# megapose6d/megapose6d

Measured on NVIDIA H100. Metric: pose hypotheses/sec through render+coarse+5x refine, higher is better.
Workload: dtype f16

## Files before the change

### include/mpx.h

```cpp
#ifndef MPX_H_
#define MPX_H_

#include <stddef.h>
#include <stdint.h>

#ifdef __cplusplus
extern "C" {
#endif

#define MPX_ABI_VERSION 5

int mpx_abi_version(void);
int mpx_act_dtype(void);
const char* mpx_last_error(void);
long long mpx_launch_count(void);
int mpx_set_sm_limit(int n_sms);
int mpx_sm_count(void);
int mpx_profile_enable(int on);
int mpx_profile_summary(double* conv_ms, double* conv_flops, long long* conv_launches);

typedef struct mpx_meshdb mpx_meshdb;
int mpx_meshdb_create(int n_meshes, const float* h_verts, const float* h_normals,
                      const float* h_colors, const int64_t* h_vert_offsets, const int32_t* h_faces,
                      const int64_t* h_face_offsets, mpx_meshdb** out);
// ... 37 lines not shown
                          int c_in, void* d_x, int c_pad, int ch_per_view, const float* d_depth_norm_z,
                          void* d_workspace, size_t workspace_bytes, void* stream);

int mpx_pose_init_autodepth(const float* d_points, int n_pts, const int32_t* d_label_idx,
                            const float* d_bboxes, const float* d_K, const float* d_R, int n,
                            float* d_TCO, void* stream);

int mpx_normalize_T(const float* d_T_in, int n, float* d_T_out, void* stream);

int mpx_crop_geometry(const float* d_points, int n_pts, const int32_t* d_label_idx,
                      const float* d_TCO, const float* d_K, const float* d_tCR, int n, float lamb,
                      int im_h, int im_w, int out_h, int out_w, float* d_boxes_rend,
                      float* d_boxes_crop, float* d_K_crop, void* stream);

int mpx_multiview_cameras(const float* d_TCO, const float* d_tCR, int n, const float* h_offsets,
                          int n_extra, float* d_TCV_O, void* stream);

int mpx_pose_update(const float* d_TCO, const float* d_K_crop, const float* d_pose9,
                    const float* d_tCR, int n, float* d_TCO_out, void* stream);

int mpx_topk_per_group(const float* d_logits, int n_groups, int m, int k, int32_t* d_idx,
                       void* stream);

int mpx_image_to_nhwc4(const float* d_images_nchw, int b, int c, int h, int w, float* d_out_nhwc4,
                       void* stream);
int mpx_roi_align(const float* d_img_nhwc4, int b, int h, int w, const int32_t* d_im_idx,
                  const float* d_boxes, int n, int c, int out_h, int out_w, float* d_out,
                  void* stream);
int mpx_roi_align_fused(const float* d_img_nhwc4, int b, int h, int w, const int32_t* d_im_idx,
                        const float* d_boxes, int n, int c, int out_h, int out_w, void* d_x,
                        int c_pad, const float* d_depth_norm_z, int depth_norm_kind, void* stream);

size_t mpx_net_input_bytes(int n, int h, int w, int c_pad);

int mpx_conv2d(const void* d_x, int n, int h, int w, int c_in, const void* d_w,
                    const float* d_bias, int c_out, int r, int s, int stride, int pad_lo_h,
                    int pad_lo_w, int pad_hi_h, int pad_hi_w, int relu, const void* d_residual,
                    void* d_out, int block_n, int max_ctas, void* stream);

int mpx_conv2d_splitk(const void* d_x, int n, int h, int w, int c_in, const void* d_w,
                           const float* d_bias, int c_out, int r, int s, int stride, int pad_lo_h,
                           int pad_lo_w, int pad_hi_h, int pad_hi_w, int relu, const void* d_residual,
                           void* d_out, int block_n, int splits, void* stream);

#define MPX_CONV_NET_SPLITK 8
#define MPX_CONV_NO_PDL 512
#define MPX_CONV_SPLITK_CAP2 262144
#define MPX_CONV_SPLITK_CAP1 524288
#define MPX_CONV_NEVER_C64 4194304
#define MPX_CONV_FORCE_IM2COL 8388608
#define MPX_CONV_FORCE_C64 67108864
#define MPX_CONV_NEVER_PP 134217728
#define MPX_CONV_FORCE_PP 268435456
int mpx_conv_set_mode(int mode);

int mpx_maxpool3x3s2(const void* d_x, int n, int h, int w, int c, void* d_out, void* stream);

int mpx_avgpool_linear(const void* d_x, int n, int hw, int c, const float* d_w, const float* d_b,
                       int out_dim, float* d_out, void* stream);

typedef struct mpx_net mpx_net;
int mpx_net_create(int c_pad, int out_dim, const void* const* h_conv_w, const float* const* h_conv_b,
                   int n_convs, const float* d_head_w, const float* d_head_b, mpx_net** out);
int mpx_net_create_preact(int c_pad, int out_dim, const int32_t* h_layer_blocks, const void* const* h_conv_w,
                          const float* const* h_conv_b, int n_convs, const float* const* h_block_affine, int n_blocks,
                          const float* d_head_w, const float* d_head_b, mpx_net** out);
int mpx_net_destroy(mpx_net* net);
int mpx_net_set_graphs(int on);
size_t mpx_net_workspace_bytes(const mpx_net* net, int n, int h, int w);
int mpx_net_forward(const mpx_net* net, const void* d_x, int n, int h, int w, float* d_out,
                    void* d_workspace, size_t workspace_bytes, void* stream);

typedef struct mpx_fpn mpx_fpn;
int mpx_fpn_create(const void* const* h_conv_w, const float* const* h_conv_b, int n_convs, int n_anchors, mpx_fpn** out);
int mpx_fpn_destroy(mpx_fpn* fpn);
size_t mpx_fpn_workspace_bytes(int n, int h, int w);
int mpx_fpn_forward(const mpx_fpn* fpn, const float* d_images, int n, int h, int w, float* const* h_features,
                    float* const* h_objectness, float* const* h_deltas, void* d_workspace, size_t workspace_bytes,
                    void* stream);

int mpx_mask_paste(const float* d_logits, const int64_t* d_labels, const float* d_boxes, int n_masks, int n_classes,
                   int m, int n_images, const int32_t* h_counts, const int32_t* h_sizes, float* d_boxes_out,
                   float* const* h_masks, void* stream);

#define MPX_BOP_MAX_TAUS 16
int mpx_bop_vsd(int n_pairs, int h, int w, const uint16_t* d_depth_test, int n_img, const float* d_depth_scale,
                const double* d_K, const float* d_depth_est, int n_est, const float* d_depth_gt, int n_gt,
                const int32_t* d_est_idx, const int32_t* d_gt_idx, const int32_t* d_img_idx, const double* d_diameter,
                const double* h_taus, int n_taus, float delta, int64_t* d_counts, double* d_err, void* stream);

#define MPX_BOP_MSSD 0
#define MPX_BOP_MSPD 1
#define MPX_BOP_ADD 2
#define MPX_BOP_ADI 3
int mpx_bop_point_errors(int kind, int n_pairs, int n_models, const double* d_pts, const int64_t* d_pt_offsets,
                         long long n_pts_total, const double* d_syms, const int64_t* d_sym_offsets, long long n_syms_total,
                         const int32_t* d_model_idx, const double* d_pose_est, const double* d_pose_gt, const double* d_K,
                         double* d_err, int32_t* d_sym_argmin, void* stream);

int mpx_bop_gt_info(int n_gt, int h, int w, const uint16_t* d_depth_test, int n_img, const float* d_depth_scale,
                    const double* d_K, const float* d_depth_gt_large, const int32_t* d_img_idx, float delta,
                    int64_t* d_counts, int32_t* d_bbox, uint8_t* d_mask, uint8_t* d_mask_visib, void* stream);

int mpx_bop_cus(int n_pairs, int h, int w, const float* d_depth_est, int n_est, const float* d_depth_gt, int n_gt,
                const int32_t* d_est_idx, const int32_t* d_gt_idx, int64_t* d_counts, double* d_err, void* stream);

// ... 35 lines not shown
```

### megapose6d_b200/csrc/conv_wgmma.cu

```cuda
#include <cuda.h>
#include <vector>
#include "mpx_common.cuh"

namespace mpx {

#ifdef MPX_ACT_BF16
#define kTmaActType CU_TENSOR_MAP_DATA_TYPE_BFLOAT16
#define MPX_WGMMA_AB "bf16.bf16"
#else
#define kTmaActType CU_TENSOR_MAP_DATA_TYPE_FLOAT16
#define MPX_WGMMA_AB "f16.f16"
#endif

__device__ __forceinline__ void mbar_init(uint64_t* bar, uint32_t count) {
  asm volatile("mbarrier.init.shared::cta.b64 [%0], %1;" ::"r"(smem_u32(bar)), "r"(count));
}
__device__ __forceinline__ void mbar_expect_tx(uint64_t* bar, uint32_t bytes) {
  asm volatile("mbarrier.arrive.expect_tx.shared::cta.b64 _, [%0], %1;" ::"r"(smem_u32(bar)), "r"(bytes) : "memory");
}
__device__ __forceinline__ void mbar_arrive(uint64_t* bar) {
  asm volatile("mbarrier.arrive.shared::cta.b64 _, [%0];" ::"r"(smem_u32(bar)) : "memory");
}
__device__ __forceinline__ bool mbar_try_wait(uint64_t* bar, uint32_t parity) {
  uint32_t ok;
// ... 381 lines not shown
          if (res_row) {
            const float2 r = unpack_act2(__ldg(reinterpret_cast<const uint32_t*>(res_row + 8 * j)));
            f0 += r.x;
            f1 += r.y;
          }
          if (p.relu) {
            f0 = fmaxf(f0, 0.f);
            f1 = fmaxf(f1, 0.f);
          }
          packed[j] = pack_act2(f0, f1);
        }
#pragma unroll
        for (int j = 0; j < BLOCK_N / 8; ++j) *reinterpret_cast<uint32_t*>(p.out + off + 8 * j) = packed[j];
      }
    }
  }

  __syncthreads();
  if (p.splits > 1) {
    cluster_sync_all();
    const int item = blockIdx.x;
    const int tile = item / p.splits;
    const int m_tile = tile / p.n_tiles;
    const int n_tile = tile - m_tile * p.n_tiles;
    const int n0 = n_tile * BLOCK_N;
    splitk_reduce_slice<BLOCK_N>(smem_u32(smem), p.splits, static_cast<int>(cluster_ctarank()),
                                 static_cast<long long>(m_tile) * kBlockM, p.M_total, p.C_out, n0, p.out, p.residual,
                                 bias_s + n0, p.relu, threadIdx.x, blockDim.x);
    cluster_sync_all();
  }
}

constexpr int kC64Pixels = 256;
constexpr int kC64Stages = 4;
constexpr int kC64ActBytes = kC64Pixels * kBlockK * 2;
constexpr int kC64WBytes = 64 * kBlockK * 2;
constexpr int kC64StageBytes = kC64ActBytes + kC64WBytes;
constexpr int kC64StagingBytes = kC64Pixels * 64 * 2;
constexpr int kC64BandSlots = 3;
constexpr int kC64BandWStages = 8;
static_assert(kC64BandSlots * kC64ActBytes + kC64BandWStages * kC64WBytes == kC64Stages * kC64StageBytes,
              "conv64: the band producer's ring layout is the im2col producer's");
constexpr int kC64SmemBytes = 227 * 1024;
constexpr int kC64BufferBytes = kC64SmemBytes - 1024  - 256  - 256 ;
static_assert(kC64Stages * kC64StageBytes + 2 * kC64StagingBytes <= kC64BufferBytes, "conv64: shared memory budget");

struct Conv64Params {
  int M_total, P, Q, S, stride, pad_h, pad_w, cblocks, num_k_blocks, m_tiles;
  int band_w, band_rows, tiles_per_img;
  int band_slots, slot_bytes, w_resident, w_off, staging_off, staging_bytes;
  int relu;
  int has_residual;
  const float* bias;
};

__device__ __forceinline__ void tma_store_2d(const CUtensorMap* map, const void* smem, int c0, int c1) {
  asm volatile("cp.async.bulk.tensor.2d.global.shared::cta.bulk_group [%0, {%2, %3}], [%1];" ::"l"(map),
               "r"(smem_u32(smem)), "r"(c0), "r"(c1)
               : "memory");
}
__device__ __forceinline__ void tma_load_4d(void* smem, const CUtensorMap* map, uint64_t* bar, int c0, int c1, int c2,
                                            int c3) {
  asm volatile(
      "cp.async.bulk.tensor.4d.shared::cluster.global.tile.mbarrier::complete_tx::bytes"
      " [%0], [%1, {%3, %4, %5, %6}], [%2];" ::"r"(smem_u32(smem)),
      "l"(map), "r"(smem_u32(bar)), "r"(c0), "r"(c1), "r"(c2), "r"(c3)
      : "memory");
}
__device__ __forceinline__ void tma_store_4d(const CUtensorMap* map, const void* smem, int c0, int c1, int c2, int c3) {
  asm volatile("cp.async.bulk.tensor.4d.global.shared::cta.bulk_group [%0, {%2, %3, %4, %5}], [%1];" ::"l"(map),
               "r"(smem_u32(smem)), "r"(c0), "r"(c1), "r"(c2), "r"(c3)
               : "memory");
}
__device__ __forceinline__ void bulk_commit() { asm volatile("cp.async.bulk.commit_group;" ::: "memory"); }
__device__ __forceinline__ void bulk_wait_read_all() { asm volatile("cp.async.bulk.wait_group.read 0;" ::: "memory"); }
__device__ __forceinline__ void bulk_wait_all() { asm volatile("cp.async.bulk.wait_group 0;" ::: "memory"); }
__device__ __forceinline__ void fence_proxy_async_smem() { asm volatile("fence.proxy.async.shared::cta;" ::: "memory"); }
__device__ __forceinline__ void warpgroup_sync(int cw) { asm volatile("bar.sync %0, 128;" ::"r"(2 + cw) : "memory"); }
__device__ __forceinline__ void mainloop_turn_wait(int cw) { asm volatile("bar.sync %0, 256;" ::"r"(4 + cw) : "memory"); }
__device__ __forceinline__ void mainloop_turn_pass(int cw) { asm volatile("bar.arrive %0, 256;" ::"r"(5 - cw) : "memory"); }

__host__ __device__ __forceinline__ uint32_t stem_live_steps(int kb, int cblocks, int S) {
  const int tap = kb / cblocks, cb = kb - tap * cblocks;
  const int r = tap / S, s = tap - r * S;
  uint32_t live = 0;
  for (int k = 0; k < 4; ++k) {
    const int slice = (4 * cb + k) / cblocks;
    const int ky = 2 * r + (slice >> 1) - 1, kx = 2 * s + (slice & 1) - 1;
    if (ky >= 0 && ky <= 6 && kx >= 0 && kx <= 6) live |= 1u << k;
  }
  return live;
}

template <int N>
__device__ __forceinline__ void wgmma_kblock(uint32_t live, float (&acc)[N / 2], uint64_t da, uint64_t db) {
  wgmma_fence();
#pragma unroll
  for (int k = 0; k < kBlockK / 16; ++k)
    if (live & (1u << k)) wgmma_tile<N>(acc, da + static_cast<uint64_t>(2 * k), db + static_cast<uint64_t>(2 * k), 1u);
  wgmma_commit();
}

template <int kStemCblocks, int kBandN>
__global__ void __launch_bounds__(kThreads, 1)
conv64_wgmma_kernel(const __grid_constant__ CUtensorMap map_x, const __grid_constant__ CUtensorMap map_w,
                    const __grid_constant__ CUtensorMap map_res, const __grid_constant__ CUtensorMap map_out,
                    const Conv64Params p) {
  constexpr bool kBand = kBandN > 0;
  constexpr int kN = kBand ? kBandN : kC64Pixels;
  constexpr int kStages = kBand ? kC64BandWStages : kC64Stages;
  extern __shared__ uint8_t smem_raw[];
  uint8_t* smem = reinterpret_cast<uint8_t*>((reinterpret_cast<uintptr_t>(smem_raw) + 1023) &
                                             ~static_cast<uintptr_t>(1023));
  uint8_t* smem_x = smem;
  uint8_t* smem_w = smem + (kBand ? p.w_off : kC64Stages * kC64ActBytes);
  uint8_t* staging = smem + (kBand ? p.staging_off : kC64Stages * kC64StageBytes);
  const int staging_bytes = kBand ? p.staging_bytes : kC64StagingBytes;
  const int slot_bytes = kBand ? p.slot_bytes : kC64ActBytes;
  const bool w_resident = kBand && p.w_resident;
  uint64_t* bars = reinterpret_cast<uint64_t*>(smem + kC64BufferBytes);
  uint64_t* full_bar = bars;
  uint64_t* empty_bar = bars + 8;
  uint64_t* res_bar = bars + 16;
  uint64_t* band_full = bars + 18;
  uint64_t* band_empty = bars + 21;
  uint64_t* w_bar = bars + 24;
  float* bias_s = reinterpret_cast<float*>(bars + 32);

  const int wg = __shfl_sync(0xffffffffu, threadIdx.x >> 7, 0);
  const int nk = p.num_k_blocks;
  for (int i = threadIdx.x; i < 64; i += blockDim.x) bias_s[i] = p.bias[i];
  if (threadIdx.x == 0) {
    asm volatile("prefetch.tensormap [%0];" ::"l"(&map_x) : "memory");
    asm volatile("prefetch.tensormap [%0];" ::"l"(&map_w) : "memory");
    asm volatile("prefetch.tensormap [%0];" ::"l"(&map_out) : "memory");
    if (p.has_residual) asm volatile("prefetch.tensormap [%0];" ::"l"(&map_res) : "memory");
    for (int i = 0; i < kStages; ++i) {
      mbar_init(&full_bar[i], 1);
      mbar_init(&empty_bar[i], 4);
    }
    if constexpr (kBand) {
      for (int i = 0; i < kC64BandSlots; ++i) {
        mbar_init(&band_full[i], 1);
        mbar_init(&band_empty[i], 4);
      }
      mbar_init(w_bar, 1);
    }
    mbar_init(&res_bar[0], 1);
    mbar_init(&res_bar[1], 1);
    asm volatile("fence.mbarrier_init.release.cluster;" ::: "memory");
  }
  pdl_trigger();
  __syncthreads();
  pdl_wait();

  if (wg == 0) {
    asm volatile("setmaxnreg.dec.sync.aligned.u32 40;");
    if (threadIdx.x == 0) {
      int stage = 0;
      uint32_t phase = 0;
      if constexpr (kBand) {
        int slot = 0;
        uint32_t slot_phase = 0;
        const uint32_t band_bytes = static_cast<uint32_t>(p.band_w * p.band_rows) * 128u;
        if (w_resident) {
          mbar_expect_tx(w_bar, static_cast<uint32_t>(nk) * kC64WBytes);
          for (int kb = 0; kb < nk; ++kb)
            tma_load_2d(smem_w + kb * kC64WBytes, &map_w, w_bar, kb * kBlockK, 0);
        }
        for (int tile = blockIdx.x; tile < p.m_tiles; tile += gridDim.x) {
          const int img = tile / p.tiles_per_img;
          const int p0 = (tile - img * p.tiles_per_img) * p.band_rows;
          int r = 0, s = 0, cb = 0;
          for (int kb = 0; kb < nk; ++kb) {
            if (s == 0) {
              mbar_wait(&band_empty[slot], slot_phase ^ 1u);
              mbar_expect_tx(&band_full[slot], band_bytes);
              tma_load_4d(smem_x + slot * slot_bytes, &map_x, &band_full[slot], cb * kBlockK, -p.pad_w,
                          p0 + r - p.pad_h, img);
              if (++slot == p.band_slots) {
                slot = 0;
                slot_phase ^= 1u;
              }
            }
            if (!w_resident) {
              mbar_wait(&empty_bar[stage], phase ^ 1u);
              mbar_expect_tx(&full_bar[stage], kC64WBytes);
              tma_load_2d(smem_w + stage * kC64WBytes, &map_w, &full_bar[stage], kb * kBlockK, 0);
              if (++stage == kStages) {
// ... 18 lines not shown
          const bool second = m0 + kBlockM < p.M_total;
#pragma unroll
          for (int hh = 0; hh < 2; ++hh) {
            const int m = m0 + hh * kBlockM;
            img[hh] = m / pq;
            const int rem = m - img[hh] * pq;
            const int p0 = rem / p.Q;
            base_w[hh] = (rem - p0 * p.Q) * p.stride - p.pad_w;
            base_h[hh] = p0 * p.stride - p.pad_h;
          }
          const uint32_t bytes = (second ? kC64ActBytes : kC64ActBytes / 2) + kC64WBytes;
          int tap = 0, cb = 0;
          for (int kb = 0; kb < nk; ++kb) {
            mbar_wait(&empty_bar[stage], phase ^ 1u);
            mbar_expect_tx(&full_bar[stage], bytes);
            const int r = tap / p.S;
            const int s = tap - r * p.S;
            uint8_t* dst = smem_x + stage * kC64ActBytes;
            tma_load_im2col_4d(dst, &map_x, &full_bar[stage], cb * kBlockK, base_w[0], base_h[0], img[0],
                               static_cast<uint16_t>(s), static_cast<uint16_t>(r));
            if (second)
              tma_load_im2col_4d(dst + kATileBytes, &map_x, &full_bar[stage], cb * kBlockK, base_w[1], base_h[1], img[1],
                                 static_cast<uint16_t>(s), static_cast<uint16_t>(r));
            tma_load_2d(smem_w + stage * kC64WBytes, &map_w, &full_bar[stage], kb * kBlockK, 0);
            if (++cb == p.cblocks) {
              cb = 0;
              ++tap;
            }
            if (++stage == kStages) {
              stage = 0;
              phase ^= 1u;
            }
          }
        }
      }
    }
  } else {
    asm volatile("setmaxnreg.inc.sync.aligned.u32 232;");
    const int cw = wg - 1;
    const int t = threadIdx.x & 127;
    const int lane = threadIdx.x & 31;
    const int q = lane >> 2;
    const int c = 16 * (t >> 5) + (q & ~1);
    const int px = 2 * (lane & 3) + (q & 1);
    const bool odd = (q & 1) != 0;
    uint8_t* stage_buf = staging + cw * staging_bytes;
    if (w_resident) mbar_wait(w_bar, 0);
    const int bands_per_tile = nk / p.S;
    int local = 0;
    for (int i = cw, tile = blockIdx.x + cw * gridDim.x; tile < p.m_tiles; i += 2, tile += 2 * gridDim.x, ++local) {
      const int m0 = tile * kC64Pixels;
      const int img = kBand ? tile / p.tiles_per_img : 0;
      const int p0 = kBand ? (tile - img * p.tiles_per_img) * p.band_rows : 0;
      if (p.has_residual && t == 0) {
        bulk_wait_read_all();
        if constexpr (kBand) {
          mbar_expect_tx(&res_bar[cw], static_cast<uint32_t>(p.band_rows * p.Q) * 128u);
          tma_load_4d(stage_buf, &map_res, &res_bar[cw], 0, 0, p0, img);
        } else {
          mbar_expect_tx(&res_bar[cw], kC64StagingBytes);
          tma_load_2d(stage_buf, &map_res, &res_bar[cw], 0, m0);
        }
      }
      const uint32_t g = static_cast<uint32_t>(i) * static_cast<uint32_t>(nk);
      int stage = static_cast<int>(g % kStages);
      uint32_t phase = (g / kStages) & 1u;
      const uint64_t gb0 = static_cast<uint64_t>(i) * static_cast<uint64_t>(bands_per_tile);
      const int slot0 = kBand ? static_cast<int>(gb0 % static_cast<uint64_t>(p.band_slots)) : 0;
      const uint32_t slot_phase0 = kBand ? static_cast<uint32_t>(gb0 / static_cast<uint64_t>(p.band_slots)) & 1u : 0u;
      float acc[kN / 2];
#pragma unroll
      for (int j = 0; j < kN / 2; ++j) acc[j] = 0.f;
      if (i > 0) mainloop_turn_wait(cw);
      int prev_stage = -1, prev_slot = -1;
      auto kblock = [&](uint32_t live, int kb, int r, int s, int cb) {
        uint64_t db;
        int slot = -1;
        if constexpr (kBand) {
          const int u = slot0 + r * p.cblocks + cb;
          slot = u % p.band_slots;
          if (s == 0) mbar_wait(&band_full[slot], slot_phase0 ^ (static_cast<uint32_t>(u / p.band_slots) & 1u));
          db = make_sw128_desc(smem_u32(smem_x + slot * slot_bytes) + static_cast<uint32_t>(s) * 128u);
        } else {
          db = make_sw128_desc(smem_u32(smem_x + stage * kC64ActBytes));
        }
        uint32_t wa;
        if (w_resident) {
          wa = smem_u32(smem_w + kb * kC64WBytes);
        } else {
          mbar_wait(&full_bar[stage], phase);
          wa = smem_u32(smem_w + stage * kC64WBytes);
        }
        wgmma_kblock<kN>(live, acc, make_sw128_desc(wa), db);
        wgmma_wait<1>();
        __syncwarp();
        if (prev_stage >= 0 && lane == 0) mbar_arrive(&empty_bar[prev_stage]);
        if (prev_slot >= 0 && lane == 0) mbar_arrive(&band_empty[prev_slot]);
        prev_slot = (kBand && s == p.S - 1) ? slot : -1;
        if (!w_resident) {
          prev_stage = stage;
          if (++stage == kStages) {
            stage = 0;
            phase ^= 1u;
          }
        }
      };
      if constexpr (kStemCblocks > 0) {
#pragma unroll
        for (int kb = 0; kb < 16 * kStemCblocks; ++kb)
          kblock(stem_live_steps(kb, kStemCblocks, 4), kb, kb / (4 * kStemCblocks), (kb / kStemCblocks) % 4,
                 kb % kStemCblocks);
      } else {
        int r = 0, s = 0, cb = 0;
#pragma unroll 1
        for (int kb = 0; kb < nk; ++kb) {
          kblock(0xFu, kb, r, s, cb);
          if (++cb == p.cblocks) {
            cb = 0;
            if (++s == p.S) {
              s = 0;
              ++r;
            }
          }
        }
      }
      if (tile + static_cast<int>(gridDim.x) < p.m_tiles) mainloop_turn_pass(cw);
      wgmma_wait<0>();
      __syncwarp();
      if (lane == 0) {
        if (prev_stage >= 0) mbar_arrive(&empty_bar[prev_stage]);
        if (prev_slot >= 0) mbar_arrive(&band_empty[prev_slot]);
      }

      if (t == 0) bulk_wait_read_all();
      warpgroup_sync(cw);
      if (p.has_residual) mbar_wait(&res_bar[cw], static_cast<uint32_t>(local) & 1u);
      const uint32_t sbase = smem_u32(stage_buf);
      const float2 bias2[2] = {*reinterpret_cast<const float2*>(bias_s + c), *reinterpret_cast<const float2*>(bias_s + c + 8)};
      const int rows = kBand ? min(p.band_rows, p.P - p0) : 0;
      int prow = 0, pcol = px;
#pragma unroll
      for (int j = 0; j < kN / 8; ++j) {
        if constexpr (kBand) {
          while (pcol >= p.band_w) {
            pcol -= p.band_w;
            ++prow;
          }
        }
        const bool keep = !kBand || (pcol < p.Q && prow < rows);
        const int srow = kBand ? prow * p.Q + pcol : 8 * j + px;
#pragma unroll
        for (int h = 0; h < 2; ++h) {
          const float v0 = acc[4 * j + 2 * h], v1 = acc[4 * j + 2 * h + 1];
          const float other = __shfl_xor_sync(0xffffffffu, odd ? v0 : v1, 4);
          float f0 = (odd ? other : v0) + bias2[h].x;
          float f1 = (odd ? v1 : other) + bias2[h].y;
          const int chunk = (c + 8 * h) >> 3;
          const uint32_t addr = sbase + static_cast<uint32_t>(srow * 128 + ((chunk ^ (srow & 7)) << 4) + ((c & 7) << 1));
          if (keep) {
            if (p.has_residual) {
              uint32_t rr;
              asm volatile("ld.shared.b32 %0, [%1];" : "=r"(rr) : "r"(addr) : "memory");
              const float2 r = unpack_act2(rr);
              f0 += r.x;
              f1 += r.y;
            }
            if (p.relu) {
              f0 = fmaxf(f0, 0.f);
              f1 = fmaxf(f1, 0.f);
            }
            asm volatile("st.shared.b32 [%0], %1;" ::"r"(addr), "r"(pack_act2(f0, f1)) : "memory");
          }
        }
        pcol += 8;
      }
      fence_proxy_async_smem();
      warpgroup_sync(cw);
      if (t == 0) {
        if constexpr (kBand) tma_store_4d(&map_out, stage_buf, 0, 0, p0, img);
        else tma_store_2d(&map_out, stage_buf, 0, m0);
        bulk_commit();
      }
    }
    if (t == 0) bulk_wait_all();
  }
}

constexpr int kPPStages = 4;
constexpr int kPPStageBytes = 2 * kATileBytes;
constexpr int kPPStagingBytes = kBlockM * 128 * 2;
constexpr int kPPBufferBytes = kPPStages * kPPStageBytes + 2 * kPPStagingBytes;
constexpr int kPPSmemBytes = kPPBufferBytes + 1024  + 256  + 2048 ;

struct ConvPPParams {
  int P, Q, S, stride, pad_h, pad_w, cblocks, num_k_blocks, m_tiles, n_tiles;
  int relu;
  int has_residual;
  const float* bias;
};

__global__ void __launch_bounds__(kThreads, 1)
convpp_wgmma_kernel(const __grid_constant__ CUtensorMap map_a, const __grid_constant__ CUtensorMap map_b,
                    const __grid_constant__ CUtensorMap map_res, const __grid_constant__ CUtensorMap map_out,
                    const ConvPPParams p) {
  extern __shared__ uint8_t smem_raw[];
  uint8_t* smem = reinterpret_cast<uint8_t*>((reinterpret_cast<uintptr_t>(smem_raw) + 1023) &
                                             ~static_cast<uintptr_t>(1023));
  uint8_t* smem_a = smem;
  uint8_t* smem_b = smem + kPPStages * kATileBytes;
  uint8_t* staging = smem + kPPStages * kPPStageBytes;
  uint64_t* bars = reinterpret_cast<uint64_t*>(smem + kPPBufferBytes);
  uint64_t* full_bar = bars;
  uint64_t* empty_bar = bars + 8;
  uint64_t* res_bar = bars + 16;
  float* bias_s = reinterpret_cast<float*>(bars + 32);

  const int wg = __shfl_sync(0xffffffffu, threadIdx.x >> 7, 0);
  const int nk = p.num_k_blocks;
  const int items = p.m_tiles * p.n_tiles;
  for (int i = threadIdx.x; i < 128 * p.n_tiles; i += blockDim.x) bias_s[i] = p.bias[i];
  if (threadIdx.x == 0) {
    asm volatile("prefetch.tensormap [%0];" ::"l"(&map_a) : "memory");
    asm volatile("prefetch.tensormap [%0];" ::"l"(&map_b) : "memory");
    asm volatile("prefetch.tensormap [%0];" ::"l"(&map_out) : "memory");
    if (p.has_residual) asm volatile("prefetch.tensormap [%0];" ::"l"(&map_res) : "memory");
    for (int i = 0; i < kPPStages; ++i) {
      mbar_init(&full_bar[i], 1);
      mbar_init(&empty_bar[i], 4);
    }
    mbar_init(&res_bar[0], 1);
    mbar_init(&res_bar[1], 1);
    asm volatile("fence.mbarrier_init.release.cluster;" ::: "memory");
  }
  pdl_trigger();
// ... 242 lines not shown
                              CU_TENSOR_MAP_INTERLEAVE_NONE, CU_TENSOR_MAP_SWIZZLE_128B, CU_TENSOR_MAP_L2_PROMOTION_L2_128B,
                              CU_TENSOR_MAP_FLOAT_OOB_FILL_NONE);
  MPX_REQUIRE(r == CUDA_SUCCESS, "cuTensorMapEncodeTiled failed (%d)", static_cast<int>(r));
  return MPX_OK;
}

static bool conv64_band_fits(const ConvDesc& d) {
  const int wp = d.W + d.pad_lo_w + d.pad_hi_w;
  return d.stride == 1 && wp <= kC64Pixels && d.C_in / kBlockK <= kC64BandSlots - 1;
}

static void conv64_band_layout(Conv64Params& p, int band_n, int S) {
  auto round1k = [](int b) { return (b + 1023) & ~1023; };
  const int slot = round1k(p.band_w * p.band_rows * 128);
  const int staging = round1k(p.band_rows * p.Q * 128);
  const int weights = p.num_k_blocks * kC64WBytes;
  const int reach = (band_n + S - 2) * 128 + 128;
  for (int slots = kC64BandSlots; slots >= p.cblocks + 1; --slots) {
    const int end = slots * slot + weights + 2 * staging;
    if (end <= kC64BufferBytes && (slots - 1) * slot + reach <= kC64BufferBytes) {
      p.band_slots = slots;
      p.slot_bytes = slot;
      p.w_resident = 1;
      p.w_off = slots * slot;
      p.staging_off = p.w_off + weights;
      p.staging_bytes = staging;
      return;
    }
  }
  p.band_slots = kC64BandSlots;
  p.slot_bytes = kC64ActBytes;
  p.w_resident = 0;
  p.w_off = kC64BandSlots * kC64ActBytes;
  p.staging_off = p.w_off + kC64BandWStages * kC64WBytes;
  p.staging_bytes = kC64StagingBytes;
}

static int conv64_forward(const ConvDesc& d, const void* x, const void* w, const float* bias, const void* residual,
                          void* out, int M_total, int P, int Q, int cap, cudaStream_t stream) {
  const int K_total = d.R * d.S * d.C_in;
  Conv64Params p{};
  p.M_total = M_total;
  p.P = P;
  p.Q = Q;
  p.S = d.S;
  p.stride = d.stride;
  p.pad_h = d.pad_lo_h;
  p.pad_w = d.pad_lo_w;
  p.cblocks = d.C_in / kBlockK;
  p.num_k_blocks = d.R * d.S * p.cblocks;
  p.relu = d.relu;
  p.has_residual = residual != nullptr;
  p.bias = bias;
  const bool band = conv64_band_fits(d) && (g_conv_mode & MPX_CONV_FORCE_IM2COL) == 0;
  int band_n = 0;
  CUtensorMap map_x, map_w, map_res, map_out;
  int rc;
  if (band) {
    p.band_w = d.W + d.pad_lo_w + d.pad_hi_w;
    p.band_rows = kC64Pixels / p.band_w < P ? kC64Pixels / p.band_w : P;
    p.tiles_per_img = (P + p.band_rows - 1) / p.band_rows;
    p.m_tiles = d.n_img * p.tiles_per_img;
    band_n = (p.band_rows - 1) * p.band_w + Q <= 160 ? 160 : 256;
    conv64_band_layout(p, band_n, d.S);
    rc = encode_nhwc_map(&map_x, x, d.n_img, d.H, d.W, d.C_in, p.band_w, p.band_rows);
    if (rc != MPX_OK) return rc;
    rc = encode_nhwc_map(&map_out, out, d.n_img, P, Q, 64, Q, p.band_rows);
    if (rc != MPX_OK) return rc;
    map_res = map_out;
    if (residual != nullptr) {
      rc = encode_nhwc_map(&map_res, residual, d.n_img, P, Q, 64, Q, p.band_rows);
      if (rc != MPX_OK) return rc;
    }
  } else {
    p.m_tiles = (M_total + kC64Pixels - 1) / kC64Pixels;
    rc = encode_im2col_map(&map_x, d, x);
    if (rc != MPX_OK) return rc;
    rc = encode_2d_map(&map_out, out, 64, M_total, 64, kC64Pixels, CU_TENSOR_MAP_L2_PROMOTION_L2_128B);
    if (rc != MPX_OK) return rc;
    map_res = map_out;
    if (residual != nullptr) {
      rc = encode_2d_map(&map_res, residual, 64, M_total, 64, kC64Pixels, CU_TENSOR_MAP_L2_PROMOTION_L2_128B);
      if (rc != MPX_OK) return rc;
    }
  }
  rc = encode_2d_map(&map_w, w, K_total, 64, kBlockK, 64, CU_TENSOR_MAP_L2_PROMOTION_L2_256B);
  if (rc != MPX_OK) return rc;
  const int stem_cblocks = (d.s2d_stem && d.R == 4 && d.S == 4 && p.cblocks <= 2) ? p.cblocks : 0;
  long long live_steps = 0;
  for (int kb = 0; kb < p.num_k_blocks; ++kb)
    live_steps += __builtin_popcount(stem_cblocks ? stem_live_steps(kb, p.cblocks, p.S) : 0xFu);

  typedef void (*Conv64Kernel)(CUtensorMap, CUtensorMap, CUtensorMap, CUtensorMap, Conv64Params);
  static const Conv64Kernel kernels[3][3] = {
      {conv64_wgmma_kernel<0, 0>, conv64_wgmma_kernel<0, 160>, conv64_wgmma_kernel<0, 256>},
      {conv64_wgmma_kernel<1, 0>, conv64_wgmma_kernel<1, 160>, conv64_wgmma_kernel<1, 256>},
      {conv64_wgmma_kernel<2, 0>, conv64_wgmma_kernel<2, 160>, conv64_wgmma_kernel<2, 256>}};
  static bool attr_set = false;
  if (!attr_set) {
    for (int a = 0; a < 3; ++a)
      for (int b = 0; b < 3; ++b)
        MPX_CHECK_CUDA(cudaFuncSetAttribute(kernels[a][b], cudaFuncAttributeMaxDynamicSharedMemorySize, kC64SmemBytes));
    attr_set = true;
  }
  const int grid = p.m_tiles < cap ? p.m_tiles : cap;
  ProfileSlot* slot = profile_begin(stream);
  const Conv64Kernel kernel = kernels[stem_cblocks][band_n == 0 ? 0 : (band_n == 160 ? 1 : 2)];
  MPX_CHECK_CUDA(launch_pdl(kernel, dim3(grid), dim3(kThreads), kC64SmemBytes, stream, 1, map_x, map_w, map_res, map_out,
                            p));
  MPX_CHECK_CUDA(cudaGetLastError());
  ++g_launches;
  profile_end(slot, stream, 2.0 * M_total * 64 * live_steps * 16);
  return MPX_OK;
}

static int convpp_forward(const ConvDesc& d, const void* x, const void* w, const float* bias, const void* residual,
                          void* out, int M_total, int P, int Q, int cap, cudaStream_t stream) {
  ConvPPParams p{};
  p.P = P;
  p.Q = Q;
  p.S = d.S;
  p.stride = d.stride;
  p.pad_h = d.pad_lo_h;
  p.pad_w = d.pad_lo_w;
  p.cblocks = d.C_in / kBlockK;
  p.num_k_blocks = d.R * d.S * p.cblocks;
  p.m_tiles = (M_total + kBlockM - 1) / kBlockM;
  p.n_tiles = d.C_out / 128;
  p.relu = d.relu;
  p.has_residual = residual != nullptr;
  p.bias = bias;
  CUtensorMap map_a, map_b, map_res, map_out;
  int rc = encode_im2col_map(&map_a, d, x);
  if (rc != MPX_OK) return rc;
  rc = encode_2d_map(&map_b, w, static_cast<cuuint64_t>(p.num_k_blocks) * kBlockK, d.C_out, kBlockK, 128,
                     CU_TENSOR_MAP_L2_PROMOTION_L2_256B);
  if (rc != MPX_OK) return rc;
  rc = encode_2d_map(&map_out, out, d.C_out, M_total, 64, kBlockM, CU_TENSOR_MAP_L2_PROMOTION_L2_128B);
  if (rc != MPX_OK) return rc;
  map_res = map_out;
  if (residual != nullptr) {
    rc = encode_2d_map(&map_res, residual, d.C_out, M_total, 64, kBlockM, CU_TENSOR_MAP_L2_PROMOTION_L2_128B);
    if (rc != MPX_OK) return rc;
  }
  static bool attr_set = false;
  if (!attr_set) {
    MPX_CHECK_CUDA(cudaFuncSetAttribute(convpp_wgmma_kernel, cudaFuncAttributeMaxDynamicSharedMemorySize, kPPSmemBytes));
    attr_set = true;
  }
  const int items = p.m_tiles * p.n_tiles;
  const int grid = items < cap ? items : cap;
  ProfileSlot* slot = profile_begin(stream);
  MPX_CHECK_CUDA(launch_pdl(convpp_wgmma_kernel, dim3(grid), dim3(kThreads), kPPSmemBytes, stream, 1, map_a, map_b,
                            map_res, map_out, p));
  MPX_CHECK_CUDA(cudaGetLastError());
  ++g_launches;
  profile_end(slot, stream, 2.0 * M_total * d.C_out * p.num_k_blocks * kBlockK);
  return MPX_OK;
}

int conv_forward(const ConvDesc& d, const void* x, const void* w, const float* bias,
                 const void* residual, void* out, int block_n_override, int max_ctas,
                 cudaStream_t stream, int splitk, int max_c_out) {
  MPX_REQUIRE(d.C_in % 64 == 0 && d.C_in >= 64, "conv: C_in=%d must be a multiple of 64", d.C_in);
  MPX_REQUIRE(max_c_out <= 2048, "conv: C_out limit %d above 2048", max_c_out);
  MPX_REQUIRE(d.C_out % 64 == 0 && d.C_out <= max_c_out, "conv: C_out=%d must be a multiple of 64, at most %d", d.C_out,
              max_c_out);
  MPX_REQUIRE(d.stride == 1 || d.stride == 2, "conv: stride %d unsupported", d.stride);
  MPX_REQUIRE(d.R >= 1 && d.R <= 8 && d.S >= 1 && d.S <= 8, "conv: filter %dx%d unsupported", d.R, d.S);
  int rc = load_driver_entry_points();
  if (rc != MPX_OK) return rc;

  const int P = conv_out_dim(d.H, d.pad_lo_h, d.pad_hi_h, d.R, d.stride);
  const int Q = conv_out_dim(d.W, d.pad_lo_w, d.pad_hi_w, d.S, d.stride);
  MPX_REQUIRE(P > 0 && Q > 0, "conv: empty output");
  const long long M_total = static_cast<long long>(d.n_img) * P * Q;
  MPX_REQUIRE(M_total > 0 && M_total < (1LL << 31), "conv: M=%lld out of range", M_total);

  int block_n = block_n_override;
  if (block_n <= 0) {
    const long long m_tiles_est = (M_total + kBlockM - 1) / kBlockM;
    block_n = d.C_out % 256 == 0 ? 256 : (d.C_out % 128 == 0 ? 128 : 64);
    while (block_n > 64 && m_tiles_est * (d.C_out / block_n) < 32) block_n /= 2;
  }
  MPX_REQUIRE((block_n == 64 || block_n == 128 || block_n == 256) && d.C_out % block_n == 0,
              "conv: BLOCK_N=%d invalid for C_out=%d", block_n, d.C_out);

  const bool aligned = (reinterpret_cast<uintptr_t>(out) & 15) == 0 && (reinterpret_cast<uintptr_t>(residual) & 15) == 0;
  const long long tiles256 = (M_total + kC64Pixels - 1) / kC64Pixels;
  const int cap = max_ctas > 0 ? max_ctas : sm_count();
  if (d.C_out == 64 && block_n_override == 0 && splitk <= 0 && aligned && (g_conv_mode & MPX_CONV_NEVER_C64) == 0 &&
      ((g_conv_mode & MPX_CONV_FORCE_C64) != 0 || tiles256 >= 2LL * cap)) {
    const long long m_tiles128 = (M_total + kBlockM - 1) / kBlockM;
    const int nkb = d.R * d.S * (d.C_in / kBlockK);
    if (!(splitk < 0 && m_tiles128 * 2 <= cap && nkb >= 8))
      return conv64_forward(d, x, w, bias, residual, out, static_cast<int>(M_total), P, Q, cap, stream);
  }

  const long long m_tiles = (M_total + kBlockM - 1) / kBlockM;
  if (d.C_out % 128 == 0 && d.C_out <= 512 && block_n_override == 0 && splitk <= 0 && aligned &&
      (g_conv_mode & MPX_CONV_NEVER_PP) == 0 &&
      ((g_conv_mode & MPX_CONV_FORCE_PP) != 0 || (d.C_out == 128 && m_tiles >= 2LL * cap))) {
    const int nkb = d.R * d.S * (d.C_in / kBlockK);
    if (!(splitk < 0 && m_tiles * (d.C_out / block_n) * 2 <= cap && nkb >= 8))
      return convpp_forward(d, x, w, bias, residual, out, static_cast<int>(M_total), P, Q, cap, stream);
  }

  CUtensorMap map_a, map_b;
  rc = encode_im2col_map(&map_a, d, x);
  if (rc != MPX_OK) return rc;
  rc = encode_2d_map(&map_b, w, static_cast<cuuint64_t>(d.R) * d.S * d.C_in, d.C_out, kBlockK, block_n,
                     CU_TENSOR_MAP_L2_PROMOTION_L2_256B);
  if (rc != MPX_OK) return rc;

  ConvParams p{};
  p.M_total = static_cast<int>(M_total);
  p.P = P;
  p.Q = Q;
  p.C_out = d.C_out;
  p.S = d.S;
  p.stride = d.stride;
  p.pad_h = d.pad_lo_h;
  p.pad_w = d.pad_lo_w;
  p.cblocks = d.C_in / kBlockK;
  p.num_k_blocks = d.R * d.S * p.cblocks;
  p.m_tiles = static_cast<int>((M_total + kBlockM - 1) / kBlockM);
  p.n_tiles = d.C_out / block_n;
  p.relu = d.relu;
  p.bias = bias;
  p.residual = reinterpret_cast<const act_t*>(residual);
  p.out = reinterpret_cast<act_t*>(out);
  p.splits = 1;
  if (splitk != 0) {
    const int tiles = p.m_tiles * p.n_tiles;
    const int sms = max_ctas > 0 ? max_ctas : sm_count();
    int want = splitk > 0 ? splitk : 1;
    if (splitk < 0 && tiles * 2 <= sms && p.num_k_blocks >= 8) {
      want = p.num_k_blocks / 4;
      if (want > sms / tiles) want = sms / tiles;
    }
    const int cap = (splitk < 0 && (g_conv_mode & MPX_CONV_SPLITK_CAP1))
                        ? 1
                        : ((splitk < 0 && (g_conv_mode & MPX_CONV_SPLITK_CAP2)) ? 2 : 8);
    int splits = 1;
    while (splits * 2 <= want && splits * 2 <= cap && splits * 2 <= p.num_k_blocks) splits *= 2;
// ... 15 lines not shown
```

### megapose6d_b200/csrc/mpx_common.cuh

```cuda
#pragma once
#include <cuda_runtime.h>
#include <cuda_bf16.h>
#include <cuda_fp16.h>
#include <stdint.h>
#include <stdio.h>
#include <string.h>

#include "../../include/mpx.h"

namespace mpx {

void set_error(const char* fmt, ...);

#define MPX_OK 0
#define MPX_ERR_INVALID -1
#define MPX_ERR_CUDA -2
#define MPX_ERR_UNSUPPORTED -3

#define MPX_CHECK_CUDA(expr)                                                          \
  do {                                                                                \
    cudaError_t _e = (expr);                                                          \
    if (_e != cudaSuccess) {                                                          \
      mpx::set_error("%s:%d CUDA error %s: %s", __FILE__, __LINE__, #expr,            \
                     cudaGetErrorString(_e));                                         \
// ... 75 lines not shown
#endif

__device__ __forceinline__ float depth_norm(float d, float z, int kind) {
  if (kind == 0) return fminf(fmaxf(__fdiv_rn(d, z), 0.f), 2.f) - 1.f;
  if (kind == 1) return __fdiv_rn(d, z);
  if (kind == 2) return fminf(fmaxf(d - z, -2.f), 2.f);
  return d;
}

__device__ __forceinline__ void pdl_trigger() { asm volatile("griddepcontrol.launch_dependents;" ::: "memory"); }
__device__ __forceinline__ void pdl_wait() { asm volatile("griddepcontrol.wait;" ::: "memory"); }
int conv_get_mode();
template <typename... KArgs, typename... Args>
inline cudaError_t launch_pdl(void (*kernel)(KArgs...), dim3 grid, dim3 block, size_t smem, cudaStream_t stream,
                              int cluster_x, Args&&... args) {
  cudaLaunchConfig_t cfg = {};
  cfg.gridDim = grid;
  cfg.blockDim = block;
  cfg.dynamicSmemBytes = smem;
  cfg.stream = stream;
  cudaLaunchAttribute attr[2];
  int n = 0;
  if (cluster_x > 1) {
    attr[n].id = cudaLaunchAttributeClusterDimension;
    attr[n].val.clusterDim.x = cluster_x;
    attr[n].val.clusterDim.y = 1;
    attr[n].val.clusterDim.z = 1;
    ++n;
  }
  if ((conv_get_mode() & MPX_CONV_NO_PDL) == 0) {
    attr[n].id = cudaLaunchAttributeProgrammaticStreamSerialization;
    attr[n].val.programmaticStreamSerializationAllowed = 1;
    ++n;
  }
  cfg.attrs = attr;
  cfg.numAttrs = n;
  return cudaLaunchKernelEx(&cfg, kernel, static_cast<KArgs>(args)...);
}

extern long long g_launches;
void conv_profile_enable(int on);
bool conv_profile_enabled();
void net_set_graphs(int on);
void conv_set_mode(int mode);
int conv_get_mode();
int conv_profile_summary(double* total_ms, double* total_flops, long long* launches);

struct ConvDesc {
  int n_img, H, W, C_in;
  int C_out, R, S, stride;
  int pad_lo_h, pad_lo_w, pad_hi_h, pad_hi_w;
  int relu;
  int s2d_stem;
};
int conv_forward(const ConvDesc& d, const void* x, const void* w, const float* bias,
                 const void* residual, void* out, int block_n_override, int max_ctas,
                 cudaStream_t stream, int splitk = 0, int max_c_out = 512);
int conv_out_dim(int in, int pad_lo, int pad_hi, int k, int stride);
int maxpool3x3s2(const void* x, int n, int h, int w, int c, void* out, cudaStream_t stream);
int avgpool_linear(const void* x, int n, int hw, int c, const float* w, const float* b, int out_dim,
                   float* out, cudaStream_t stream);
struct Net;
int net_create(int c_pad, int out_dim, const void* const* conv_w, const float* const* conv_b,
               int n_convs, const float* head_w, const float* head_b, Net** out);
int net_create_preact(int c_pad, int out_dim, const int* layer_blocks, const void* const* conv_w, const float* const* conv_b,
                      int n_convs, const float* const* block_affine, int n_blocks, const float* head_w, const float* head_b,
                      Net** out);
size_t net_workspace_bytes(const Net* net, int n, int h, int w);
int net_forward(const Net* net, const void* x, int n, int h, int w, float* out, void* workspace,
                size_t workspace_bytes, cudaStream_t stream);
void net_destroy(Net* net);
bool net_graphs_enabled();

struct Fpn;
constexpr int kFpnConvs = 63;
int fpn_create(const void* const* conv_w, const float* const* conv_b, int n_convs, int n_anchors, Fpn** out);
void fpn_destroy(Fpn* fpn);
size_t fpn_workspace_bytes(int n, int h, int w);
int fpn_forward(Fpn* fpn, const float* images, int n, int h, int w, float* const* features, float* const* objectness,
                float* const* deltas, void* workspace, size_t workspace_bytes, cudaStream_t stream);
constexpr int kMaskMaxImages = 64;
constexpr int kMaskMaxM = 64;
int mask_paste(const float* logits, const long long* labels, const float* boxes, int n_masks, int n_classes, int m,
               int n_images, const int* counts, const int* sizes, float* boxes_out, float* const* masks,
               cudaStream_t stream);

struct MeshDb {
  int n_meshes;
  int nv_max;
  float* verts;
  float* normals;
  float* colors;
  int* faces;
  long long* vert_offsets;
  long long* face_offsets;
  int4* vtx_cache;
  int slots;
  int nf_max;
  int4* faces4;
  float4* vattr;
  float* radius;
  unsigned* tile_scratch;
  long long tile_words;
  float* uv;
  unsigned char* tex;
  long long* tex_offsets;
  int4* tex_info;
// ... 90 lines not shown
```

### megapose6d_b200/csrc/net.cu

```cuda
#include <cuda.h>
#include <cstdlib>
#include <vector>
#include "mpx_common.cuh"

namespace mpx {


__global__ void __launch_bounds__(512)
maxpool3x3s2_kernel(const uint4* __restrict__ x, uint4* __restrict__ out, int n, int h, int w, int c8, int ho, int wo) {
  pdl_trigger();
  pdl_wait();
  const int row_items = wo * c8;
  for (int row = blockIdx.x; row < n * ho; row += gridDim.x) {
    const int img = row / ho, oy = row - img * ho;
    const int iy0 = oy * 2 - 1;
    const uint4* xin = x + static_cast<size_t>(img) * h * w * c8;
    uint4* orow = out + static_cast<size_t>(row) * row_items;
    for (int t = threadIdx.x; t < row_items; t += blockDim.x) {
      const int ox = t / c8, cc = t - ox * c8;
      const int ix0 = ox * 2 - 1;
      float m[8];
#pragma unroll
      for (int j = 0; j < 8; ++j) m[j] = -INFINITY;
#pragma unroll
// ... 264 lines not shown
    if (g.x == x && g.out == out && g.ws == workspace && g.n == n && g.h == h && g.w == w) e = &g;
  if (!e) {
    if (net->graphs.size() >= 32) {
      for (auto& g : net->graphs)
        if (g.exec) cudaGraphExecDestroy(g.exec);
      net->graphs.clear();
    }
    net->graphs.push_back(GraphEntry{x, out, workspace, n, h, w, 0, nullptr});
    e = &net->graphs.back();
  }
  if (e->exec == nullptr) {
    if (e->warm == 0) {
      e->warm = 1;
      return net_forward_direct(net, x, n, h, w, out, workspace, workspace_bytes, stream);
    }
    if (!net->side) {
      MPX_CHECK_CUDA(cudaStreamCreateWithFlags(&net->side, cudaStreamNonBlocking));
      MPX_CHECK_CUDA(cudaEventCreateWithFlags(&net->ev_in, cudaEventDisableTiming));
      MPX_CHECK_CUDA(cudaEventCreateWithFlags(&net->ev_out, cudaEventDisableTiming));
    }
    cudaGraph_t graph = nullptr;
    MPX_CHECK_CUDA(cudaStreamBeginCapture(net->side, cudaStreamCaptureModeThreadLocal));
    const long long launches_before = g_launches;
    int rc = net_forward_direct(net, x, n, h, w, out, workspace, workspace_bytes, net->side);
    cudaError_t ce = cudaStreamEndCapture(net->side, &graph);
    e->warm = static_cast<int>(g_launches - launches_before);
    g_launches = launches_before;
    if (rc != MPX_OK || ce != cudaSuccess || graph == nullptr) {
      if (graph) cudaGraphDestroy(graph);
      cudaGetLastError();
      g_use_graphs = false;
      return net_forward_direct(net, x, n, h, w, out, workspace, workspace_bytes, stream);
    }
    ce = cudaGraphInstantiate(&e->exec, graph, 0);
    cudaGraphDestroy(graph);
    if (ce != cudaSuccess) {
      e->exec = nullptr;
      cudaGetLastError();
      g_use_graphs = false;
      return net_forward_direct(net, x, n, h, w, out, workspace, workspace_bytes, stream);
    }
  }
  MPX_CHECK_CUDA(cudaEventRecord(net->ev_in, stream));
  MPX_CHECK_CUDA(cudaStreamWaitEvent(net->side, net->ev_in, 0));
  MPX_CHECK_CUDA(cudaGraphLaunch(e->exec, net->side));
  MPX_CHECK_CUDA(cudaEventRecord(net->ev_out, net->side));
  MPX_CHECK_CUDA(cudaStreamWaitEvent(stream, net->ev_out, 0));
  g_launches += e->warm;
  return MPX_OK;
}

static int stem_and_pool(const ConvDesc& d, const void* x, const void* w, const float* b, void* buf_stem, void* buf_pool,
                         cudaStream_t stream) {
  const int rc = conv_forward(d, x, w, b, nullptr, buf_stem, 0, 0, stream);
  if (rc != MPX_OK) return rc;
  return maxpool3x3s2(buf_stem, d.n_img, d.H, d.W, d.C_out, buf_pool, stream);
}

static int net_forward_preact(const Net* net, const void* x, int n, int h, int w, float* out, void* workspace,
                              cudaStream_t stream) {
  const int hs = h / 2, ws = w / 2;
  const int hp = (hs + 2 - 3) / 2 + 1, wp = (ws + 2 - 3) / 2 + 1;
  uint8_t* base = reinterpret_cast<uint8_t*>(workspace);
  const size_t stem_bytes = align256(static_cast<size_t>(n) * hs * ws * 64 * 2);
  const size_t buf_bytes = rotating_buffer_bytes(n, hp, wp);
  void* buf_stem = base;
  void* bufs[5];
  for (int i = 0; i < 5; ++i) bufs[i] = base + stem_bytes + i * buf_bytes;
  const int sk = ((conv_get_mode() & MPX_CONV_NET_SPLITK) != 0 && n <= 64) ? -1 : 0;
  int rc;
  {
    ConvDesc d{n, hs, ws, 4 * net->c_pad, 64, 3, 3, 1, 1, 1, 1, 1, 1, 0};
    rc = stem_and_pool(d, x, net->conv_w[0], net->conv_b[0], buf_stem, bufs[0], stream);
    if (rc != MPX_OK) return rc;
  }
  int ci = 1, blk_id = 0;
  int cur = 0;
  int H = hp, W = wp, C = 64;
  for (int layer = 0; layer < 4; ++layer) {
    const int width = kLayerWidth[layer];
    for (int blk = 0; blk < net->layer_blocks[layer]; ++blk, ++blk_id) {
      const int stride = (blk == 0 && layer > 0) ? 2 : 1;
      const bool has_ds = (blk == 0 && layer > 0);
      const int ia = (cur + 1) % 5, iy = (cur + 2) % 5, ir = (cur + 3) % 5, io = (cur + 4) % 5;
      const int Ho = conv_out_dim(H, 1, 1, 3, stride), Wo = conv_out_dim(W, 1, 1, 3, stride);
      rc = affine_relu(bufs[cur], static_cast<long long>(n) * H * W * C, C, net->block_affine[blk_id], bufs[ia], stream);
      if (rc != MPX_OK) return rc;
      ConvDesc d1{n, H, W, C, width, 3, 3, stride, 1, 1, 1, 1, 1, 0};
      rc = conv_forward(d1, bufs[ia], net->conv_w[ci], net->conv_b[ci], nullptr, bufs[iy], 0, 0, stream, sk);
      if (rc != MPX_OK) return rc;
      const void* residual = bufs[cur];
      if (has_ds) {
        ConvDesc dd{n, H, W, C, width, 1, 1, stride, 0, 0, 0, 0, 0, 0};
        rc = conv_forward(dd, bufs[ia], net->conv_w[ci + 2], net->conv_b[ci + 2], nullptr, bufs[ir], 0, 0, stream, sk);
        if (rc != MPX_OK) return rc;
        residual = bufs[ir];
      }
      ConvDesc d2{n, Ho, Wo, width, width, 3, 3, 1, 1, 1, 1, 1, 0, 0};
      rc = conv_forward(d2, bufs[iy], net->conv_w[ci + 1], net->conv_b[ci + 1], residual, bufs[io], 0, 0, stream, sk);
      if (rc != MPX_OK) return rc;
      ci += has_ds ? 3 : 2;
      cur = io;
      H = Ho;
      W = Wo;
      C = width;
    }
// ... 80 lines not shown
```

Baseline: 29570.

## Fuse stem 3x3/s2 maxpool into conv64 band epilogue via global red.max

```diff
diff --git a/include/mpx.h b/include/mpx.h
--- a/include/mpx.h
+++ b/include/mpx.h
@@ -113,6 +113,7 @@
 #define MPX_CONV_FORCE_C64 67108864
 #define MPX_CONV_NEVER_PP 134217728
 #define MPX_CONV_FORCE_PP 268435456
+#define MPX_CONV_UNFUSED_POOL 536870912
 int mpx_conv_set_mode(int mode);
 
 int mpx_maxpool3x3s2(const void* d_x, int n, int h, int w, int c, void* d_out, void* stream);
diff --git a/megapose6d_b200/csrc/conv_wgmma.cu b/megapose6d_b200/csrc/conv_wgmma.cu
--- a/megapose6d_b200/csrc/conv_wgmma.cu
+++ b/megapose6d_b200/csrc/conv_wgmma.cu
@@ -457,6 +457,7 @@
   int relu;
   int has_residual;
   const float* bias;
+  act_t* pooled;
 };
 
 __device__ __forceinline__ void tma_store_2d(const CUtensorMap* map, const void* smem, int c0, int c1) {
@@ -497,6 +498,22 @@
   return live;
 }
 
+__device__ __forceinline__ void red_max_act8(act_t* dst, const uint32_t (&v)[4]) {
+#ifdef MPX_ACT_BF16
+  asm volatile("red.global.max.noftz.v4.bf16x2 [%0], {%1, %2, %3, %4};" ::"l"(dst), "r"(v[0]), "r"(v[1]), "r"(v[2]),
+               "r"(v[3])
+               : "memory");
+#else
+  asm volatile("red.global.max.noftz.v4.f16x2 [%0], {%1, %2, %3, %4};" ::"l"(dst), "r"(v[0]), "r"(v[1]), "r"(v[2]),
+               "r"(v[3])
+               : "memory");
+#endif
+}
+__device__ __forceinline__ uint32_t max_act2(uint32_t a, uint32_t b) {
+  const act_t2 r = __hmax2(*reinterpret_cast<const act_t2*>(&a), *reinterpret_cast<const act_t2*>(&b));
+  return *reinterpret_cast<const uint32_t*>(&r);
+}
+
 template <int N>
 __device__ __forceinline__ void wgmma_kblock(uint32_t live, float (&acc)[N / 2], uint64_t da, uint64_t db) {
   wgmma_fence();
@@ -512,7 +529,8 @@
                     const __grid_constant__ CUtensorMap map_res, const __grid_constant__ CUtensorMap map_out,
                     const Conv64Params p) {
   constexpr bool kBand = kBandN > 0;
-  constexpr int kN = kBand ? kBandN : kC64Pixels;
+  constexpr bool kPool = (kBandN & 1) != 0;
+  constexpr int kN = kBand ? kBandN - kPool : kC64Pixels;
   constexpr int kStages = kBand ? kC64BandWStages : kC64Stages;
   extern __shared__ uint8_t smem_raw[];
   uint8_t* smem = reinterpret_cast<uint8_t*>((reinterpret_cast<uintptr_t>(smem_raw) + 1023) &
@@ -539,7 +557,7 @@
     asm volatile("prefetch.tensormap [%0];" ::"l"(&map_x) : "memory");
     asm volatile("prefetch.tensormap [%0];" ::"l"(&map_w) : "memory");
     asm volatile("prefetch.tensormap [%0];" ::"l"(&map_out) : "memory");
-    if (p.has_residual) asm volatile("prefetch.tensormap [%0];" ::"l"(&map_res) : "memory");
+    if (!kPool && p.has_residual) asm volatile("prefetch.tensormap [%0];" ::"l"(&map_res) : "memory");
     for (int i = 0; i < kStages; ++i) {
       mbar_init(&full_bar[i], 1);
       mbar_init(&empty_bar[i], 4);
@@ -664,7 +682,7 @@
       const int m0 = tile * kC64Pixels;
       const int img = kBand ? tile / p.tiles_per_img : 0;
       const int p0 = kBand ? (tile - img * p.tiles_per_img) * p.band_rows : 0;
-      if (p.has_residual && t == 0) {
+      if (!kPool && p.has_residual && t == 0) {
         bulk_wait_read_all();
         if constexpr (kBand) {
           mbar_expect_tx(&res_bar[cw], static_cast<uint32_t>(p.band_rows * p.Q) * 128u);
@@ -746,7 +764,7 @@
 
       if (t == 0) bulk_wait_read_all();
       warpgroup_sync(cw);
-      if (p.has_residual) mbar_wait(&res_bar[cw], static_cast<uint32_t>(local) & 1u);
+      if (!kPool && p.has_residual) mbar_wait(&res_bar[cw], static_cast<uint32_t>(local) & 1u);
       const uint32_t sbase = smem_u32(stage_buf);
       const float2 bias2[2] = {*reinterpret_cast<const float2*>(bias_s + c), *reinterpret_cast<const float2*>(bias_s + c + 8)};
       const int rows = kBand ? min(p.band_rows, p.P - p0) : 0;
@@ -770,7 +788,7 @@
           const int chunk = (c + 8 * h) >> 3;
           const uint32_t addr = sbase + static_cast<uint32_t>(srow * 128 + ((chunk ^ (srow & 7)) << 4) + ((c & 7) << 1));
           if (keep) {
-            if (p.has_residual) {
+            if (!kPool && p.has_residual) {
               uint32_t rr;
               asm volatile("ld.shared.b32 %0, [%1];" : "=r"(rr) : "r"(addr) : "memory");
               const float2 r = unpack_act2(rr);
@@ -786,12 +804,44 @@
         }
         pcol += 8;
       }
-      fence_proxy_async_smem();
-      warpgroup_sync(cw);
-      if (t == 0) {
-        if constexpr (kBand) tma_store_4d(&map_out, stage_buf, 0, 0, p0, img);
-        else tma_store_2d(&map_out, stage_buf, 0, m0);
-        bulk_commit();
+      if constexpr (kPool) {
+        warpgroup_sync(cw);
+        const int pp = (p.P - 1) / 2 + 1, pq = (p.Q - 1) / 2 + 1;
+        const int chunk = t & 7;
+        const int last = p0 + rows - 1;
+        const int py_end = min((last + 1) >> 1, pp - 1);
+        for (int py = p0 >> 1; py <= py_end; ++py) {
+          act_t* prow = p.pooled + (static_cast<size_t>(img) * pp + py) * pq * 64 + chunk * 8;
+          for (int px = t >> 3; px < pq; px += 16) {
+            uint32_t m[4] = {0u, 0u, 0u, 0u};
+#pragma unroll
+            for (int dy = 0; dy < 3; ++dy) {
+              const int ys = 2 * py - 1 + dy - p0;
+              if (ys < 0 || ys >= rows) continue;
+#pragma unroll
+              for (int dx = 0; dx < 3; ++dx) {
+                const int xs = 2 * px - 1 + dx;
+                if (xs < 0 || xs >= p.Q) continue;
+                const int srow = ys * p.Q + xs;
+                uint32_t v[4];
+                asm volatile("ld.shared.v4.b32 {%0, %1, %2, %3}, [%4];"
+                             : "=r"(v[0]), "=r"(v[1]), "=r"(v[2]), "=r"(v[3])
+                             : "r"(sbase + static_cast<uint32_t>(srow * 128 + ((chunk ^ (srow & 7)) << 4))));
+#pragma unroll
+                for (int k = 0; k < 4; ++k) m[k] = max_act2(m[k], v[k]);
+              }
+            }
+            red_max_act8(prow + static_cast<size_t>(px) * 64, m);
+          }
+        }
+      } else {
+        fence_proxy_async_smem();
+        warpgroup_sync(cw);
+        if (t == 0) {
+          if constexpr (kBand) tma_store_4d(&map_out, stage_buf, 0, 0, p0, img);
+          else tma_store_2d(&map_out, stage_buf, 0, m0);
+          bulk_commit();
+        }
       }
     }
     if (t == 0) bulk_wait_all();
@@ -1140,6 +1190,7 @@
   p.relu = d.relu;
   p.has_residual = residual != nullptr;
   p.bias = bias;
+  if (d.pool) p.pooled = reinterpret_cast<act_t*>(out);
   const bool band = conv64_band_fits(d) && (g_conv_mode & MPX_CONV_FORCE_IM2COL) == 0;
   int band_n = 0;
   CUtensorMap map_x, map_w, map_res, map_out;
@@ -1153,7 +1204,8 @@
     conv64_band_layout(p, band_n, d.S);
     rc = encode_nhwc_map(&map_x, x, d.n_img, d.H, d.W, d.C_in, p.band_w, p.band_rows);
     if (rc != MPX_OK) return rc;
-    rc = encode_nhwc_map(&map_out, out, d.n_img, P, Q, 64, Q, p.band_rows);
+    if (d.pool) map_out = map_x;
+    else rc = encode_nhwc_map(&map_out, out, d.n_img, P, Q, 64, Q, p.band_rows);
     if (rc != MPX_OK) return rc;
     map_res = map_out;
     if (residual != nullptr) {
@@ -1184,16 +1236,24 @@
       {conv64_wgmma_kernel<0, 0>, conv64_wgmma_kernel<0, 160>, conv64_wgmma_kernel<0, 256>},
       {conv64_wgmma_kernel<1, 0>, conv64_wgmma_kernel<1, 160>, conv64_wgmma_kernel<1, 256>},
       {conv64_wgmma_kernel<2, 0>, conv64_wgmma_kernel<2, 160>, conv64_wgmma_kernel<2, 256>}};
+  static const Conv64Kernel pooled_kernels[2][2] = {
+      {conv64_wgmma_kernel<1, 161>, conv64_wgmma_kernel<1, 257>},
+      {conv64_wgmma_kernel<2, 161>, conv64_wgmma_kernel<2, 257>}};
   static bool attr_set = false;
   if (!attr_set) {
     for (int a = 0; a < 3; ++a)
       for (int b = 0; b < 3; ++b)
         MPX_CHECK_CUDA(cudaFuncSetAttribute(kernels[a][b], cudaFuncAttributeMaxDynamicSharedMemorySize, kC64SmemBytes));
+    for (int a = 0; a < 2; ++a)
+      for (int b = 0; b < 2; ++b)
+        MPX_CHECK_CUDA(
+            cudaFuncSetAttribute(pooled_kernels[a][b], cudaFuncAttributeMaxDynamicSharedMemorySize, kC64SmemBytes));
     attr_set = true;
   }
   const int grid = p.m_tiles < cap ? p.m_tiles : cap;
   ProfileSlot* slot = profile_begin(stream);
-  const Conv64Kernel kernel = kernels[stem_cblocks][band_n == 0 ? 0 : (band_n == 160 ? 1 : 2)];
+  const Conv64Kernel kernel = d.pool ? pooled_kernels[stem_cblocks - 1][band_n == 160 ? 0 : 1]
+                                     : kernels[stem_cblocks][band_n == 0 ? 0 : (band_n == 160 ? 1 : 2)];
   MPX_CHECK_CUDA(launch_pdl(kernel, dim3(grid), dim3(kThreads), kC64SmemBytes, stream, 1, map_x, map_w, map_res, map_out,
                             p));
   MPX_CHECK_CUDA(cudaGetLastError());
@@ -1247,6 +1307,21 @@
   return MPX_OK;
 }
 
+static bool conv64_selected(long long M_total, int cap) {
+  const long long tiles256 = (M_total + kC64Pixels - 1) / kC64Pixels;
+  return (g_conv_mode & MPX_CONV_NEVER_C64) == 0 && ((g_conv_mode & MPX_CONV_FORCE_C64) != 0 || tiles256 >= 2LL * cap);
+}
+
+bool conv_pool_fused(const ConvDesc& d) {
+  if (!d.relu || !d.s2d_stem || d.C_out != 64 || d.R != 4 || d.S != 4 || d.C_in % kBlockK != 0 ||
+      d.C_in / kBlockK > 2 || (g_conv_mode & (MPX_CONV_UNFUSED_POOL | MPX_CONV_FORCE_IM2COL)) != 0 ||
+      !conv64_band_fits(d))
+    return false;
+  const int P = conv_out_dim(d.H, d.pad_lo_h, d.pad_hi_h, d.R, d.stride);
+  const int Q = conv_out_dim(d.W, d.pad_lo_w, d.pad_hi_w, d.S, d.stride);
+  return P > 0 && Q > 0 && conv64_selected(static_cast<long long>(d.n_img) * P * Q, sm_count());
+}
+
 int conv_forward(const ConvDesc& d, const void* x, const void* w, const float* bias,
                  const void* residual, void* out, int block_n_override, int max_ctas,
                  cudaStream_t stream, int splitk, int max_c_out) {
@@ -1275,10 +1350,14 @@
               "conv: BLOCK_N=%d invalid for C_out=%d", block_n, d.C_out);
 
   const bool aligned = (reinterpret_cast<uintptr_t>(out) & 15) == 0 && (reinterpret_cast<uintptr_t>(residual) & 15) == 0;
-  const long long tiles256 = (M_total + kC64Pixels - 1) / kC64Pixels;
   const int cap = max_ctas > 0 ? max_ctas : sm_count();
-  if (d.C_out == 64 && block_n_override == 0 && splitk <= 0 && aligned && (g_conv_mode & MPX_CONV_NEVER_C64) == 0 &&
-      ((g_conv_mode & MPX_CONV_FORCE_C64) != 0 || tiles256 >= 2LL * cap)) {
+  if (d.pool) {
+    MPX_REQUIRE(conv_pool_fused(d) && residual == nullptr && block_n_override == 0 && max_ctas == 0 && splitk == 0 &&
+                    aligned,
+                "conv: the pooled epilogue serves only the band stem (conv_pool_fused), full grid, no residual");
+    return conv64_forward(d, x, w, bias, residual, out, static_cast<int>(M_total), P, Q, cap, stream);
+  }
+  if (d.C_out == 64 && block_n_override == 0 && splitk <= 0 && aligned && conv64_selected(M_total, cap)) {
     const long long m_tiles128 = (M_total + kBlockM - 1) / kBlockM;
     const int nkb = d.R * d.S * (d.C_in / kBlockK);
     if (!(splitk < 0 && m_tiles128 * 2 <= cap && nkb >= 8))
diff --git a/megapose6d_b200/csrc/mpx_common.cuh b/megapose6d_b200/csrc/mpx_common.cuh
--- a/megapose6d_b200/csrc/mpx_common.cuh
+++ b/megapose6d_b200/csrc/mpx_common.cuh
@@ -151,7 +151,9 @@
   int pad_lo_h, pad_lo_w, pad_hi_h, pad_hi_w;
   int relu;
   int s2d_stem;
-};
+  int pool;
+};
+bool conv_pool_fused(const ConvDesc& d);
 int conv_forward(const ConvDesc& d, const void* x, const void* w, const float* bias,
                  const void* residual, void* out, int block_n_override, int max_ctas,
                  cudaStream_t stream, int splitk = 0, int max_c_out = 512);
diff --git a/megapose6d_b200/csrc/net.cu b/megapose6d_b200/csrc/net.cu
--- a/megapose6d_b200/csrc/net.cu
+++ b/megapose6d_b200/csrc/net.cu
@@ -340,6 +340,13 @@
 
 static int stem_and_pool(const ConvDesc& d, const void* x, const void* w, const float* b, void* buf_stem, void* buf_pool,
                          cudaStream_t stream) {
+  if (conv_pool_fused(d)) {
+    const int hp = (d.H - 1) / 2 + 1, wp = (d.W - 1) / 2 + 1;
+    MPX_CHECK_CUDA(cudaMemsetAsync(buf_pool, 0, static_cast<size_t>(d.n_img) * hp * wp * d.C_out * 2, stream));
+    ConvDesc dp = d;
+    dp.pool = 1;
+    return conv_forward(dp, x, w, b, nullptr, buf_pool, 0, 0, stream);
+  }
   const int rc = conv_forward(d, x, w, b, nullptr, buf_stem, 0, 0, stream);
   if (rc != MPX_OK) return rc;
   return maxpool3x3s2(buf_stem, d.n_img, d.H, d.W, d.C_out, buf_pool, stream);
```

Measured after the change: 30430 (median of 6 runs). +2.9%, better.
